# lukeshope/hipims-ocl

Hardware: AMD Instinct MI355X
Metric: Mcell-steps/sec fp64 Godunov+HLLC, 4096^2 grid, 1/2/4/8 MI355X; % HBM roofline (higher is better)
Workload: dtype f64

## Files before the change

### hipims-ocl_amd/csrc/hp_domain.hpp

```cpp
#pragma once
#include "../../include/hipims_mi.h"
#include "hp_facts.hpp"
#include "hp_plan.hpp"
#include "hp_kernels.hpp"
#include "hp_peaks.hpp"
#include "hp_probes.hpp"
#include "hp_zones.hpp"
#include "hp_overview.hpp"
#include "hp_sparse.hpp"
#include "hp_bed.hpp"
#include "hp_links.hpp"
#include "hp_soil.hpp"
#include <rccl/rccl.h>

#include <algorithm>
#include <atomic>
#include <string>
#include <vector>

using namespace hp;

namespace {

thread_local std::string g_last_error;
// ... 190 lines not shown
	uint64_t         peer_rounds = 0;
	void*            peer_state[2][2] = {{nullptr, nullptr}, {nullptr, nullptr}};
	long             peer_rows[2] = {0, 0};
	unsigned*        push_arrived = nullptr;
	bool             peer_direct = false;
	bool             push_now = false;
	unsigned long long* tail_words = nullptr;
	bool             fill_now = false;
	void*            z_state = nullptr;
	unsigned long long* haz_words = nullptr;
	unsigned         pair_gen = 0;
	void*            still_rec = nullptr;
	size_t           still_rec_slots = 0;
	int              still_rec_half = 0;
	bool             still_rec_last = false;
	uint64_t         pair_cold_starts = 0;
	hipEvent_t       tune_ev[4] = {nullptr, nullptr, nullptr, nullptr};
	int              tune_phase = 0;
	bool             tune_prefer_pairs = true;
	uint64_t         tune_next = 0;
	uint64_t         tune_samples = 0, tune_switches = 0;
	float            tune_pair_ms = 0.f, tune_single_ms = 0.f;
	uint64_t         pairs = 0;
	unsigned         single_streak = 0;
	uint64_t         flux_launches = 0, flux_launches_tailed = 0;
	bool             tail_failed = false;
	bool             strip_first = false;
	bool             tail_allowed = false;
	bool             tail_want = false;
	int              tail_fresh = 0;
	bool             tail_done = false;
	bool             spec_now = false;
	uint32_t         spec_pending = 0;
	void*            spec_state = nullptr;
	void*            spec_scalars = nullptr;
	struct { int adv_fresh; uint64_t cells_calculated, iterations; } spec_host;
	uint64_t         spec_batches = 0, spec_replays = 0;
	OutputStage      out;
	PeakTracker      peaks;
	ProbeRecorder    probes;
	ZoneRecorder     zones;
	BedShapes        beds;
	LinkStore        links;
	SoilStore        soil;
};

// ... 41 lines not shown
```

### hipims-ocl_amd/csrc/hp_engine.hip

```cpp
#include "hp_domain.hpp"
#include "hp_observers.hpp"
#include "hp_actors.hpp"
#include <hip/hip_ext.h>
#include <dlfcn.h>

#include <algorithm>
#include <cmath>
#include <cstdio>
#include <cstdlib>
#include <cstring>
#include <random>
#include <string>
#include <vector>
#include <unistd.h>

namespace {

constexpr size_t CFL_SLOT_BYTES = 1024;

struct Rccl {
	void* handle = nullptr;
	decltype(&ncclGetUniqueId)   GetUniqueId = nullptr;
	decltype(&ncclCommInitRank)  CommInitRank = nullptr;
	decltype(&ncclCommDestroy)   CommDestroy = nullptr;
// ... 7 lines not shown
	std::string path;
} g_rccl;

void peer_release(hp_domain* d);
PeerBox peer_box(hp_domain* d, bool use, long timeout_ms = 0);
PeerPush make_push(const hp_domain* d);

const PlanKnobs& plan_knobs()
{
	static const PlanKnobs knobs = [] {
		auto num = [](const char* name, int unset) { const char* e = std::getenv(name); return e ? std::atoi(e) : unset; };
		auto off = [&](const char* name) { return num(name, 1) == 0; };
		auto on = [&](const char* name) { return num(name, 0) != 0; };
		auto force = [&](const char* name) { return std::getenv(name) ? (num(name, 0) != 0 ? 1 : 0) : -1; };
		PlanKnobs k;
		k.two_step = num("HP_TWO_STEP", -1);
		k.launch_tail = !off("HP_LAUNCH_TAIL"); k.strip_reduce_always = on("HP_STRIP_REDUCE_ALWAYS");
		k.pair_bdy = !off("HP_PAIR_BDY"); k.pair_strict = !off("HP_PAIR_STRICT"); k.pair_exact = force("HP_PAIR_EXACT");
		k.pair_skip = !off("HP_PAIR_SKIP"); k.fill_after_pairs = !off("HP_FILL_AFTER_PAIRS");
		k.strict_speculate = on("HP_STRICT_SPECULATE"); k.pair_tune = !off("HP_PAIR_TUNE"); k.sweep_alternate = force("HP_SWEEP_ALTERNATE");
		k.tail_max_blocks = (unsigned)num("HP_TAIL_MAX_BLOCKS", (int)TAIL_MAX_BLOCKS);
		k.tail_max_blocks_k2k6 = (unsigned)num("HP_TAIL_MAX_BLOCKS_K2K6", (int)TAIL_MAX_BLOCKS);
		k.march2_rseg_forced = std::getenv("HP_MARCH2_RSEG") != nullptr;
		k.fuse_bdy = !off("HP_FUSE_BDY");
		return k;
	}();
	return knobs;
}
PlanDomain plan_domain(const hp_domain* d)
{
	PlanDomain p;
	p.scheme = d->desc.scheme; p.kernel = d->desc.kernel; p.math_mode = d->desc.math_mode; p.precision = d->desc.precision; p.dynamic_dt = d->desc.dynamic_dt;
	p.quirks = d->desc.quirks; p.rows = d->desc.rows; p.cols = d->desc.cols; p.cells = d->cells;
	p.row_offset = d->desc.row_offset; p.global_rows = d->desc.global_rows; p.ghost_rows = d->ghost_rows;
	p.has_bdy = !d->bdy.empty(); p.fusable = d->fusable; p.bdy_on_ring = d->bdy_on_ring;
	for (const Boundary& b : d->bdy)
		if ((b.kind == BDY_UNIFORM && b.definition == HP_UNIFORM_LOSS_RATE) || (b.kind == BDY_GRIDDED && b.definition == HP_GRIDDED_MASS_FLUX)) p.bdy_removes_water = true;
	p.has_comm = d->comm != nullptr; p.comm_world = d->comm_world; p.peer_direct = d->peer_direct; p.peer_mine = d->peer_mine != nullptr;
	p.has_tail_words = d->tail_words != nullptr; p.tail_allowed = d->tail_allowed; p.halo_overlap = d->halo_overlap; p.split_now = d->split_now;
	p.strip_any_bdy = d->strip_any_bdy; p.strip_first = d->strip_first; p.strip_any_full = d->strip_any_full;
	p.spec_now = d->spec_now; p.has_stamps = d->z_state != nullptr; p.march2_pays = d->tiling.march2_pays;
	p.has_links = d->links.groups != 0; p.soil_on = d->soil.on;
#ifdef HP_KEEP_SPEC_FUSED
	p.spec_fused_kept = true;
#endif
	return p;
}

template <typename T> Params<T> make_params(const hp_domain* d)
{
	Params<T> p;
	p.cols = d->desc.cols; p.rows = d->desc.rows;
	p.row_offset = d->desc.row_offset; p.global_rows = d->desc.global_rows;
	p.dx = (T)d->desc.dx;
	p.inv_dx = T(1) / p.dx;
	p.vs = (T)d->desc.dry_threshold;
	p.qs = (T)d->desc.dry_threshold * T(10);
	p.courant = (T)d->desc.courant;
	p.t_end = (T)d->desc.t_end;
	p.dt_fixed = (T)d->desc.dt_fixed;
	p.friction = d->desc.friction;
	p.dynamic_dt = d->desc.dynamic_dt;
	p.manning_uniform = d->manning_uniform ? 1 : 0;
	p.manning_value = (T)d->manning_value;
// ... 434 lines not shown
	const size_t slots = (size_t)windows * (size_t)d->desc.rows;
	if (d->still_rec && d->still_rec_slots == slots) return HP_OK;
	hipFree(d->still_rec);
	d->still_rec = nullptr;
	d->facts.buffers_written_outside();
	const size_t bytes = (2 * slots + 1) * sizeof(StillRec);
	HIP_TRY(hipMalloc(&d->still_rec, bytes));
	HIP_TRY(hipMemsetAsync(d->still_rec, 0xff, bytes, d->stream));
	d->still_rec_slots = slots;
	return HP_OK;
}
template <typename T> int pair_cold_start(hp_domain* d)
{
	int rc;
	d->facts.buffers_written_outside();
	if ((rc = apply_boundaries<T>(d, d->state[0])) != HP_OK) return rc;
	if ((rc = launch_reduce<T>(d, d->state[0], d->own_lo, d->own_hi)) != HP_OK) return rc;
	hipLaunchKernelGGL((pair_cold_start_words<T>), dim3(1), dim3(1), 0, d->stream, (T*)d->cfl_slot);
	HIP_TRY(hipGetLastError());
	d->facts.cold_started();
	d->pair_cold_starts++;
	return HP_OK;
}
template <typename T> int run_pair_t(hp_domain* d, const bool strip, const bool followed)
{
	const Params<T> p = make_params<T>(d);
	TileMap tm;
	unsigned blocks;
	long lo, hi;
	if (strip) {
		const bool south = d->desc.row_offset > 0, north = d->desc.row_offset + d->desc.rows < d->desc.global_rows;
		lo = south ? d->ghost_rows : 1;
		hi = d->desc.rows - (north ? d->ghost_rows : 1);
	} else launch_rows(d, 1, lo, hi);
	const PlanDomain pd = plan_domain(d);
	const PlanKnobs& knobs = plan_knobs();
	const int rseg2 = pair_tile_rows(pd, knobs, d->tiling.march2_rseg);
	if (!make_tile_map(launch_knobs(), lo, hi, 1, PART_ALL, (int)((p.cols - 2 + MARCH2_COLS - 1) / MARCH2_COLS), rseg2, rseg2, 0, tm, blocks, rseg2,
	                   0, d->own_lo, d->own_hi, d->tiling.march2_nbands))
		return HP_ERR_STATE;
	if (blocks > tail_limit(knobs)) return HP_ERR_STATE;
	d->tail_want = true; d->tail_allowed = true; d->push_now = strip;
	d->tail_fresh = strip ? (d->desc.dynamic_dt ? 7 : 4) : (d->desc.dynamic_dt ? 1 : 0);
	d->tail_done = false;
	LaunchTail<T> tail;
	const int kind = make_tail<T>(d, blocks, PART_ALL, d->stream, tail_limit(knobs), tail);
	d->tail_want = false; d->tail_allowed = false; d->push_now = false;
	if (kind != (strip ? 2 : 1)) return HP_ERR_STATE;
	const bool bdy = pd.has_bdy;
	int rc;
	if ((rc = pair_stamps_alloc(d)) != HP_OK) return rc;
	bool in_place = false;
	if (bdy && !d->facts->m1_valid) {
		if ((rc = pair_cold_start<T>(d)) != HP_OK) return rc;
		in_place = true;
	} else if (bdy) in_place = d->facts->pair_fused_next;
	tail.pair = bdy ? 2 : 1;
	tail.bdy_flag = bdy && followed ? 1 : 0;
	PairAux<T> aux{};
	const bool exact = pair_exact(pd, knobs) && d->z_state != nullptr;
	if (exact) aux.stamps = StampBufs<T>{(char*)d->z_state, d->haz_words};
	aux.prev_gen = d->facts->other_stale ? d->pair_gen : 0u;
	aux.gen = ++d->pair_gen;
	if (aux.gen == 0) aux.gen = ++d->pair_gen;
	aux.list = (const AreaBdyList<T>*)d->fused_list; aux.fuse_next = bdy && followed ? 1 : 0; aux.in_place = in_place ? 1 : 0;
	aux.truncated = (d->desc.quirks & HP_QUIRK_BDY_TRUNCATED) != 0 ? 1 : 0;
	const bool recs = pair_records(pd, knobs, strip, exact, rseg2);
	if (recs) {
		if ((rc = still_rec_alloc(d, tm.nstrips)) != HP_OK) return rc;
		StillRec* const base = (StillRec*)d->still_rec;
		aux.still_out = base + (size_t)(d->still_rec_half ^ 1) * d->still_rec_slots;
		aux.still_in = d->facts->still_rec_valid ? base + (size_t)d->still_rec_half * d->still_rec_slots : nullptr;
		aux.still_rows = d->desc.rows;
	}
	const void* src = d->state[0];
	void* dst = d->state[1];
	const bool sample = d->timing_stride > 0 && d->timing_used < d->timing_events.size() &&
	                    (d->timing_counter++ % (uint64_t)d->timing_stride) == 0;
	if (sample) HIP_TRY(hipEventRecord(d->timing_events[d->timing_used].first, d->stream));
#define HP_LAUNCH_K1B2(CFL_, BDY_, HZ_, TAIL_)                                                                                            \
	hipLaunchKernelGGL((godunov_march2<false, CFL_, BDY_, HZ_, TAIL_, T>), dim3(blocks), dim3(256), 0, d->stream, p, (const Scalars<T>*)d->scalars, \
	                   (const T*)d->bed, (const State4<T>*)src, (State4<T>*)dst, (const T*)d->manning, (T*)d->cfl_slot,                    \
	                   (const T*)d->cfl_slot + SLOT_EDGE, tm, tail, aux)
#define HP_LAUNCH_K1B(CFL_, BDY_, TAIL_) do { if (exact) HP_LAUNCH_K1B2(CFL_, BDY_, true, TAIL_); else HP_LAUNCH_K1B2(CFL_, BDY_, false, TAIL_); } while (0)
	if (d->desc.math_mode == HP_MATH_STRICT)
		hipLaunchKernelGGL((godunov_march2<true, 1, false, true, 1, T>), dim3(blocks), dim3(256), 0, d->stream, p, (const Scalars<T>*)d->scalars,
		                   (const T*)d->bed, (const State4<T>*)src, (State4<T>*)dst, (const T*)d->manning, (T*)d->cfl_slot,
		                   (const T*)d->cfl_slot + SLOT_EDGE, tm, tail, aux);
	else
	if (strip)    { if (d->desc.dynamic_dt) HP_LAUNCH_K1B2(1, false, false, 2); else HP_LAUNCH_K1B2(0, false, false, 2); }
	else if (bdy) HP_LAUNCH_K1B(1, true, 1);
	else          { if (d->desc.dynamic_dt) HP_LAUNCH_K1B(1, false, 1); else HP_LAUNCH_K1B(0, false, 1); }
#undef HP_LAUNCH_K1B
#undef HP_LAUNCH_K1B2
	d->facts.pair_queued(bdy, followed);
	HIP_TRY(hipGetLastError());
	if (recs) d->still_rec_half ^= 1;
	d->facts.pair_launched(recs); d->still_rec_last = recs;
	if (sample) { HIP_TRY(hipEventRecord(d->timing_events[d->timing_used].second, d->stream)); d->timing_used++; }
	std::swap(d->state[0], d->state[1]);
	if (strip) {
		std::swap(d->peer_state[0][0], d->peer_state[0][1]);
		std::swap(d->peer_state[1][0], d->peer_state[1][1]);
	}
	d->facts.pair_ran(strip, d->ghost_rows);
	d->single_streak = 0;
	d->tail_done = false; d->fork_is_advance = false;
	d->adv_fresh = d->desc.dynamic_dt ? 1 : 0;
	d->cells_calculated += 2 * (uint64_t)d->desc.cols * (uint64_t)d->desc.rows;
	d->iterations += 2;
	d->pairs += 1;
	return HP_OK;
}
static int run_pair(hp_domain* d, const bool strip = false, const bool followed = false)
{
	return d->desc.precision == 8 ? run_pair_t<double>(d, strip, followed) : run_pair_t<float>(d, strip, followed);
}
static int repair_other_buffer(hp_domain* d)
{
	if (!d->facts->other_stale) return HP_OK;
	d->facts.buffers_written_outside();
	HIP_TRY(hipMemcpyAsync(d->state[d->facts->use_alt ^ 1], d->state[d->facts->use_alt], d->cells * 4 * d->esize, hipMemcpyDeviceToDevice, d->stream));
	if (d->z_state) {
		if (d->desc.precision == 8)
			hipLaunchKernelGGL((stamps_to_buffer<double>), dim3(1024), dim3(256), 0, d->stream, (State4<double>*)d->state[d->facts->use_alt ^ 1],
			                   StampBufs<double>{(char*)d->z_state, d->haz_words}, d->pair_gen, d->cells);
		else
			hipLaunchKernelGGL((stamps_to_buffer<float>), dim3(1024), dim3(256), 0, d->stream, (State4<float>*)d->state[d->facts->use_alt ^ 1],
			                   StampBufs<float>{(char*)d->z_state, d->haz_words}, d->pair_gen, d->cells);
		HIP_TRY(hipGetLastError());
	}
	d->facts.other_made_current();
	return HP_OK;
}
static int snapshot_take(hp_domain* d, void* state, void* scalars, const int first)
{
	const size_t bytes = d->cells * 4 * d->esize;
	const size_t sc_bytes = d->desc.precision == 8 ? sizeof(Scalars<double>) : sizeof(Scalars<float>);
	HIP_TRY(hipMemcpyAsync(state, d->state[first], bytes, hipMemcpyDeviceToDevice, d->stream));
// ... 522 lines not shown
			if ((rc = pair_stamps_alloc(d)) != HP_OK) return rc;
			rc = run_pair(d, false, true);
			if (rc == HP_OK) {
				HIP_TRY(hipEventRecord(d->tune_ev[0], d->stream));
				if ((rc = run_pair(d, false, true)) != HP_OK || (rc = run_pair(d, false, true)) != HP_OK) return rc;
				HIP_TRY(hipEventRecord(d->tune_ev[1], d->stream));
				if ((rc = repair_other_buffer(d)) != HP_OK) return rc;
				if ((rc = run_single(d, true)) != HP_OK || (rc = run_single(d, true)) != HP_OK) return rc;
				HIP_TRY(hipEventRecord(d->tune_ev[2], d->stream));
				for (int k = 0; k < 4; ++k)
					if ((rc = run_single(d, k < 3 || i + 12 < n_iterations)) != HP_OK) return rc;
				HIP_TRY(hipEventRecord(d->tune_ev[3], d->stream));
				d->tune_phase = 1;
				i += 11;
				continue;
			}
			if (rc != HP_ERR_STATE) return rc;
		}
		if (i + 2 <= n_iterations && (!tune || d->tune_prefer_pairs) && pair_eligible(plan_domain(d), d->facts, plan_knobs())) {
			rc = run_pair(d, false, i + 2 < n_iterations);
			if (rc == HP_OK) { ++i; continue; }
			if (rc != HP_ERR_STATE) return rc;
		}
		if ((rc = run_single(d, i + 1 < n_iterations)) != HP_OK) return rc;
	}
	d->fuse_next = 0;
	return HP_OK;
}
int spec_resolve(hp_domain* d)
{
	const uint32_t n = d->spec_pending;
	d->spec_pending = 0;
	HIP_TRY(hipStreamSynchronize(d->stream));
	static const long force = std::getenv("HP_STRICT_SPEC_FORCE") ? std::atol(std::getenv("HP_STRICT_SPEC_FORCE")) : 0;
	const double flag = *(volatile double*)((char*)d->host_scalars + HOST_SPEC_FLAG);
	const bool raised = flag != 0.0 || (force > 0 && d->spec_batches % (uint64_t)force == 0);
	if (!raised) return HP_OK;
	d->spec_replays++;
	log_line(HP_LOG_INFORMATION, "a speculative STRICT batch of " + std::to_string(n) + " iterations is re-run with the plain divisions");
	const size_t bytes = d->cells * 4 * d->esize, sc_bytes = sizeof(Scalars<double>);
	d->facts.buffers_written_outside();
	HIP_TRY(hipMemcpyAsync(d->state[0], d->spec_state, bytes, hipMemcpyDeviceToDevice, d->stream));
	HIP_TRY(hipMemcpyAsync(d->state[1], (char*)d->spec_state + bytes, bytes, hipMemcpyDeviceToDevice, d->stream));
	HIP_TRY(hipMemcpyAsync(d->scalars, d->spec_scalars, sc_bytes, hipMemcpyDeviceToDevice, d->stream));
	HIP_TRY(hipMemcpyAsync(d->cfl_slot, (char*)d->spec_scalars + sc_bytes, CFL_SLOT_BYTES, hipMemcpyDeviceToDevice, d->stream));
	d->facts.spec_replayed();
// ... 722 lines not shown
	double total = 0.0;
	uint32_t n = 0;
	for (size_t i = 0; i < d->timing_used; ++i) {
		float ms = 0.f;
		HIP_TRY(hipEventElapsedTime(&ms, d->timing_events[i].first, d->timing_events[i].second));
		total += std::max(0.0, (double)ms - d->timing_overhead_ms);
		++n;
	}
	*avg_ms = n ? total / n : 0.0;
	*samples = n;
	return HP_OK;
}

int hp_pair_stats(hp_domain_t* d, uint64_t out[12])
{
	int rc = check_domain(d);
	if (rc != HP_OK) return rc;
	if (!out) return fail(HP_ERR_INVALID, "out == NULL");
	out[0] = d->pairs; out[1] = d->pair_cold_starts; out[2] = out[3] = 0;
	HIP_TRY(hipStreamSynchronize(d->stream));
	if (tuner_on(plan_domain(d), plan_knobs()) && (rc = tuner_poll(d)) != HP_OK) return rc;
	out[4] = d->tune_samples; out[5] = d->tune_switches; out[6] = d->tune_prefer_pairs ? 1 : 0;
	out[7] = d->tune_single_ms > 0.f ? (uint64_t)(1000.0 * d->tune_pair_ms / d->tune_single_ms) : 0;
	out[8] = out[9] = out[10] = out[11] = 0;
	if (d->still_rec && d->still_rec_last) {
		const StillRec* half = (const StillRec*)d->still_rec + (size_t)d->still_rec_half * d->still_rec_slots;
		unsigned long long* counts = (unsigned long long*)((StillRec*)d->still_rec + 2 * d->still_rec_slots);
		HIP_TRY(hipMemsetAsync(counts, 0, 16, d->stream));
		hipLaunchKernelGGL(still_rec_count, dim3(256), dim3(256), 0, d->stream, half, d->still_rec_slots, counts);
		HIP_TRY(hipGetLastError());
		unsigned long long host_counts[2] = {0, 0};
		HIP_TRY(hipMemcpyAsync(host_counts, counts, sizeof host_counts, hipMemcpyDeviceToHost, d->stream));
		HIP_TRY(hipStreamSynchronize(d->stream));
		out[9] = host_counts[0]; out[10] = host_counts[1];
	}
	if (d->haz_words) {
		unsigned long long used = 0;
		HIP_TRY(hipMemcpy(&used, d->haz_words + 2, sizeof used, hipMemcpyDeviceToHost));
		out[8] = used;
	}
	if (!d->z_state) return HP_OK;
	unsigned long long* counts = d->haz_words + 4;
	HIP_TRY(hipMemsetAsync(counts, 0, 16, d->stream));
	if (d->desc.precision == 8)
		hipLaunchKernelGGL((stamps_count<double>), dim3(1024), dim3(256), 0, d->stream, StampBufs<double>{(char*)d->z_state, d->haz_words}, d->pair_gen, d->cells, counts);
	else
		hipLaunchKernelGGL((stamps_count<float>), dim3(1024), dim3(256), 0, d->stream, StampBufs<float>{(char*)d->z_state, d->haz_words}, d->pair_gen, d->cells, counts);
// ... 29 lines not shown
```

### hipims-ocl_amd/csrc/hp_kernels.hpp

```cpp
#pragma once

#include "hp_math.hpp"
#include "hp_tiling.hpp"

namespace hp {

template <bool STRICT, typename T>
__global__ __launch_bounds__(256) void godunov_basic(const Params<T> p, const Scalars<T>* __restrict__ sc,
                                                     const T* __restrict__ bed, const State4<T>* __restrict__ src,
                                                     State4<T>* __restrict__ dst, const T* __restrict__ manning,
                                                     const long y_lo, const long y_hi)
{
	const long x = (long)blockIdx.x * blockDim.x + threadIdx.x;
	const long y = (long)blockIdx.y * blockDim.y + threadIdx.y + y_lo;
	if (x >= p.cols - 1 || y >= y_hi || x <= 0) return;
	const size_t id = (size_t)y * p.cols + x;
	const T dt = sc->dt;

	if (dt <= T(0)) { dst[id] = src[id]; return; }

	const State4<T> c = src[id];
	const T zb = bed[id], n = manning[id];
	if (c.zmax <= T(-9999.0) || c.z == T(-9999.0)) { dst[id] = c; return; }

// ... 836 lines not shown
				}
				if (FUSED && fuse) {
					const State4<T> rained = apply_fused(c, zb, y);
					dst[id] = rained;
					if (TAIL == 2) store_peer(rained, y, true);
				}
			}
		}
	}

	if (CFL_MODE != 0) {
		if (blockIdx.x == 0 && wave == 0) { const T e = *edge_max; if (e > vmax) vmax = e; }
		vmax = wave_max(vmax);
		if (TAIL != 0) wave_vmax = vmax;
		else if (lane == 0 && vmax > T(0)) atomic_max_nonneg(cfl_slot, vmax);
	}
	if (FUSED && blockIdx.x == 0 && wave == 0 && lane == 0) cfl_slot[SLOT_BDY] = fuse_flag ? T(1) : T(0);
	}
	if (TAIL != 0) tail_block_done(tail, wave_vmax, wave, lane, y0, y1);
}

template <typename T> struct RowU1 { State4<T> c; T zb; bool plain; };

template <bool STRICT, int CFL_MODE, bool BDY, bool HZ, int TAIL, typename T>
#ifndef HP_K1B_WAVES_MIN
#define HP_K1B_WAVES_MIN 3
#endif
#ifndef HP_K1B_F32_WAVES_MIN
#define HP_K1B_F32_WAVES_MIN 5
#endif
#ifndef HP_K1B_F32_WAVES_MAX
#define HP_K1B_F32_WAVES_MAX 5
#endif
__global__ __launch_bounds__(256) __attribute__((amdgpu_waves_per_eu(sizeof(T) == 4 ? (STRICT ? 3 : (HZ ? 4 : HP_K1B_F32_WAVES_MIN)) : (STRICT ? HP_K1B_STRICT_WAVES : HP_K1B_WAVES_MIN), sizeof(T) == 4 ? (STRICT ? 3 : HP_K1B_F32_WAVES_MAX) : (STRICT ? HP_K1B_STRICT_WAVES : 3)))) void godunov_march2(
	const Params<T> p, const Scalars<T>* sc, const T* __restrict__ bed, const State4<T>* __restrict__ src,
	State4<T>* __restrict__ dst, const T* __restrict__ manning, T* cfl_slot, const T* __restrict__ edge_max,
	const TileMap tm, const LaunchTail<T> tail, const PairAux<T> aux)
{
	if (TAIL != 0 && blockIdx.x >= tail.flux_blocks) {
		launch_tail(p, tail);
		return;
	}
	__shared__ T inc_tab[BDY ? 4 * 3 * FUSED_BDY_MAX * 2 * 64 : 1];
	const int lane = threadIdx.x & 63, wave = __builtin_amdgcn_readfirstlane((int)(threadIdx.x >> 6));
	long strip, y0, y1;
	T wave_vmax = T(0), wave_vmax1 = T(0);
	if (tile_rows(tm, wave, strip, y0, y1)) {

	const long x = strip * MARCH2_COLS - 1 + lane;
	const long xc = x < 0 ? 0 : (x < p.cols ? x : (p.cols - 1));
	const bool out_x = lane >= 2 && lane <= MARCH2_COLS + 1 && x <= p.cols - 2;
	const bool ring_x = x <= 0 || x >= p.cols - 1;
	const T vs = p.vs;
	const bool with_friction = p.friction != 0;
	const T inv_dx = STRICT ? p.inv_dx_pow2 : p.inv_dx;

	Scalars<T> s1 = *sc;
	const Scalars<T> s0 = s1;
	const T dt_a = s1.dt;
	advance_scalars(p, s1, p.dynamic_dt ? cfl_slot[BDY ? SLOT_M1 : SLOT_SAVED] : T(0));
	const T dt_b = s1.dt;
	const bool skip_a = dt_a <= T(0), skip_b = dt_b <= T(0);
	constexpr bool SCALAR_CONSTS = !STRICT && sizeof(T) == 8;
	constexpr bool HIDE = BDY || HZ;
	const StepConsts<T> ka{uniform_value<HIDE>(-(dt_a * p.inv_dx)), uniform_value<HIDE>(dt_a * gravity<T>()), SCALAR_CONSTS};
	const StepConsts<T> kb{uniform_value<HIDE>(-(dt_b * p.inv_dx)), uniform_value<HIDE>(dt_b * gravity<T>()), SCALAR_CONSTS};

	const long row_base = y0 - 2 < 0 ? 0 : y0 - 2, col_base = strip * MARCH2_COLS - 1 < 0 ? 0 : strip * MARCH2_COLS - 1;
	const size_t cell0 = (size_t)row_base * p.cols + (size_t)col_base;
	const size_t cells_left = (size_t)p.cols * p.rows - cell0;
	const __amdgpu_buffer_rsrc_t srd_src = make_srd(src + cell0, cells_left * sizeof(State4<T>));
	const __amdgpu_buffer_rsrc_t srd_dst = make_srd(dst + cell0, cells_left * sizeof(State4<T>));
	const __amdgpu_buffer_rsrc_t srd_bed = make_srd(bed + cell0, cells_left * sizeof(T));
	const __amdgpu_buffer_rsrc_t srd_man = make_srd(manning + cell0, cells_left * sizeof(T));
	const unsigned lane_col = (unsigned)(xc - col_base);
	const unsigned voff_state = lane_col * (unsigned)sizeof(State4<T>), voff_scalar = lane_col * (unsigned)sizeof(T);
	const unsigned row_state = (unsigned)p.cols * (unsigned)sizeof(State4<T>), row_scalar = (unsigned)p.cols * (unsigned)sizeof(T);
	const long last_row = p.rows - 1;
	const __amdgpu_buffer_rsrc_t srd_peer0 = make_srd((TAIL == 2 && tail.peer_rows[0] ? tail.peer_rows[0] : dst) + cell0, cells_left * sizeof(State4<T>));
	const __amdgpu_buffer_rsrc_t srd_peer1 = make_srd((TAIL == 2 && tail.peer_rows[1] ? tail.peer_rows[1] : dst) + cell0, cells_left * sizeof(State4<T>));
	auto store_peer = [&](const State4<T>& v, const long y, const bool write_lane) {
		const bool e0 = (int)y >= tail.edge_rows[0] && (int)y < tail.edge_rows[1];
		const bool e1 = (int)y >= tail.edge_rows[2] && (int)y < tail.edge_rows[3];
		buf_store_state<HP_AUX_THROUGH>(v, e1 ? srd_peer1 : srd_peer0, (write_lane && (e0 || e1)) ? voff_state : HP_OOB, (unsigned)(y - row_base) * row_state);
	};
// ... 417 lines not shown
			const unsigned row_k = (unsigned)__builtin_amdgcn_readfirstlane((int)(yy - row_base));
			buf_store_state(c, srd_dst, out_x ? voff_state : HP_OOB, row_k * row_state);
			if (TAIL == 2) store_peer(c, yy, out_x);
			if (CFL_MODE == 1 && out_x && (int)yy >= tm.price_lo && (int)yy < tm.price_hi && spd > vmax) vmax = spd;
		};
		State4<T> a = q[2].c, b = q[3].c;
		for (;;) {
			if (y >= y1) return y;
			#pragma unroll
			for (int j = 0; j < 4; ++j) q[j] = load_rz(y + 2 + j);
			if (!in_run(q[0])) return y;
			put(a, y);
			if (y + 1 >= y1 || !in_run(q[1])) return y + 1;
			put(b, y + 1);
			if (y + 2 >= y1 || !in_run(q[2])) return y + 2;
			put(q[0].c, y + 2);
			if (y + 3 >= y1 || !in_run(q[3])) return y + 3;
			put(q[1].c, y + 3);
			a = q[2].c; b = q[3].c;
			y += 4;
		}
	};

	const long yb = (RUNS && !skip_a && !skip_b) ? still_run() : y0;
	write_recs(STILL_TAG_RUN);
	if (!RUNS || yb < y1) {
		prime(yb);
		long r = yb + 1;
		for (; r + 1 <= y1; r += 2) {
			{ const T nn = rc.n; const RowU1<T> u = stage_a(r, rP, rQ); stage_b(r - 1, u, nn, true); }
			{ const T nn = rc.n; const RowU1<T> u = stage_a(r + 1, rQ, rP); stage_b(r, u, nn, true); }
		}
		if (r <= y1) { const T nn = rc.n; const RowU1<T> u = stage_a(r, rP, rQ); stage_b(r - 1, u, nn, true); }
	}

	if (wave_any(stale_rows != 0)) {
		for (long y = y0; y < y1; ++y) {
			if ((stale_rows >> (unsigned)(y - y0)) & 1u) {
				const size_t id = (size_t)y * p.cols + xc;
				const T zb = bed[id];
				State4<T> c = src[id];
				if (live0) c = apply(J0(), c, zb, y);
				State4<T> next = c;
				if (live2) next = apply(J2(), c, zb, y);
				dst[id] = fuse ? next : c;
				if (TAIL == 2) store_peer(fuse ? next : c, y, true);
				if (CFL_MODE == 1 && (int)y >= tm.price_lo && (int)y < tm.price_hi) {
					const T s = cfl_speed<STRICT>(c.z, c.zmax, c.qx, c.qy, zb, p.qs);
					if (s > vmax) vmax = s;
					if (live2) {
						const T s2 = cfl_speed<STRICT>(next.z, next.zmax, next.qx, next.qy, zb, p.qs);
						if (s2 > vmax1) vmax1 = s2;
					}
				}
			}
		}
	}
	if (!live2) vmax1 = vmax;
	};

	auto raise_word = [&]() { if (hz_on && wave_any(stamped) && lane == 0) aux.stamps.haz[aux.gen & 1u] = (unsigned long long)aux.gen; };
	if (RECS && aux.still_in != nullptr && !skip_a && !skip_b && tile_known()) {
		still_marks = ~0u;
		write_recs(STILL_TAG_SKIP);
		if (CFL_MODE == 1 && out_x && (int)y1 > tm.price_lo && (int)y0 < tm.price_hi)
			vmax = cfl_speed<STRICT>(T(__longlong_as_double((long long)still_kz)), T(0), T(0), T(0), T(__longlong_as_double((long long)still_kb)), p.qs);
		vmax1 = vmax;
	} else {
	if (BDY && act != 0) { if (hz_any) march(std::true_type(), std::true_type()); else march(std::true_type(), std::false_type()); }
	else                 { if (hz_any) march(std::false_type(), std::true_type()); else march(std::false_type(), std::false_type()); }
	raise_word();
	}

	if (CFL_MODE != 0) {
		if (blockIdx.x == 0 && wave == 0) { const T e = *edge_max; if (e > vmax) vmax = e; if (e > vmax1) vmax1 = e; }
		vmax = wave_max(vmax);
		if (BDY) vmax1 = wave_max(vmax1);
		if (TAIL != 0) { wave_vmax = vmax; wave_vmax1 = vmax1; }
		else if (lane == 0 && vmax > T(0)) atomic_max_nonneg(cfl_slot, vmax);
	}
	}
	if (TAIL != 0) tail_block_done<BDY>(tail, wave_vmax, wave, lane, y0, y1, wave_vmax1);
}

template <typename T>
__global__ __launch_bounds__(256) void stamps_to_buffer(State4<T>* __restrict__ other, const StampBufs<T> b, const unsigned gen, const size_t cells)
{
	if (b.haz[gen & 1u] != (unsigned long long)gen) return;
	for (size_t id = (size_t)blockIdx.x * blockDim.x + threadIdx.x; id < cells; id += (size_t)gridDim.x * blockDim.x)
		if (stamp_gen(b, id) == gen) other[id] = stamp_state(b, id);
}

template <typename T>
__global__ __launch_bounds__(256) void stamps_count(const StampBufs<T> b, const unsigned gen, const size_t cells, unsigned long long* counts)
{
	unsigned long long last = 0, any = 0;
	for (size_t id = (size_t)blockIdx.x * blockDim.x + threadIdx.x; id < cells; id += (size_t)gridDim.x * blockDim.x) {
		const unsigned g = stamp_gen(b, id);
		last += (g != 0 && g == gen); any += (g != 0);
	}
	for (int off = 32; off > 0; off >>= 1) { last += __shfl_down(last, off); any += __shfl_down(any, off); }
	if ((threadIdx.x & 63) == 0 && (last | any)) { atomicAdd(counts, last); atomicAdd(counts + 1, any); }
}
__global__ __launch_bounds__(256) void still_rec_count(const StillRec* __restrict__ rec, const size_t n, unsigned long long* counts)
{
// ... 636 lines not shown
```

### hipims-ocl_amd/csrc/hp_plan.hpp

```cpp
#pragma once
#include "../../include/hipims_mi.h"
#include "hp_facts.hpp"

#include <algorithm>
#include <cstddef>
#include <cstdint>

namespace hp {
namespace {

constexpr unsigned TAIL_MAX_BLOCKS = 65536;
constexpr uint32_t SPEC_MIN = 8;

struct PlanKnobs {
	int      two_step = -1;
	bool     launch_tail = true;
	bool     strip_reduce_always = false;
	bool     pair_bdy = true;
	bool     pair_strict = true;
	int      pair_exact = -1;
	bool     pair_skip = true;
	bool     fill_after_pairs = true;
	bool     strict_speculate = false;
	bool     pair_tune = true;
	int      sweep_alternate = -1;
	unsigned tail_max_blocks = TAIL_MAX_BLOCKS;
	unsigned tail_max_blocks_k2k6 = TAIL_MAX_BLOCKS;
	bool     march2_rseg_forced = false;
	bool     fuse_bdy = true;
};

struct PlanDomain {
	int      scheme = HP_SCHEME_GODUNOV, kernel = HP_KERNEL_AUTO, math_mode = HP_MATH_FAST, precision = 8, dynamic_dt = 1;
	unsigned quirks = HP_QUIRKS_REFERENCE;
	long     rows = 0, cols = 0;
	size_t   cells = 0;
	long     row_offset = 0, global_rows = 0, ghost_rows = 1;
	bool     has_bdy = false;
	bool     fusable = false, bdy_on_ring = false;
	bool     bdy_removes_water = false;
	bool     has_comm = false;
	int      comm_world = 1;
	bool     peer_direct = false, peer_mine = false;
	bool     has_tail_words = true, tail_allowed = false, halo_overlap = false, split_now = true;
	bool     strip_any_bdy = false, strip_first = false, strip_any_full = false;
	bool     spec_now = false;
	bool     has_stamps = false;
	bool     march2_pays = false;
	bool     has_links = false, soil_on = false;
	bool     spec_fused_kept = false;
};

inline bool reads_primary(const PlanDomain& d) { return (d.quirks & HP_QUIRK_CFL_READS_PRIMARY) != 0; }
inline bool basic_godunov(const PlanDomain& d) { return d.kernel == HP_KERNEL_BASIC && d.scheme == HP_SCHEME_GODUNOV; }
inline bool boundaries_applied(const PlanDomain& d) { return d.has_bdy && d.scheme != HP_SCHEME_MUSCL_HANCOCK; }

inline unsigned tail_limit(const PlanKnobs& k) { return k.tail_max_blocks < TAIL_MAX_BLOCKS ? k.tail_max_blocks : TAIL_MAX_BLOCKS; }
inline unsigned tail_limit_k2k6(const PlanKnobs& k) { return std::min(tail_limit(k), k.tail_max_blocks_k2k6); }
inline int tail_kind_for(const bool tail_want, const bool part_all, const bool own_stream, const unsigned blocks, const unsigned limit, const bool push_now)
{
	if (!(tail_want && part_all && own_stream && blocks <= limit)) return 0;
	return push_now ? 2 : 1;
}

inline bool sweep_alternates(const PlanDomain& d, const PlanKnobs& k)
{
	if (k.sweep_alternate >= 0) return k.sweep_alternate != 0;
	return d.precision == 4 || d.scheme == HP_SCHEME_MUSCL_HANCOCK;
}

inline bool pairs_possible_common(const PlanDomain& d, const PlanKnobs& k)
// ... 14 lines not shown
	       d.global_rows == d.rows;
}
inline bool pair_eligible(const PlanDomain& d, const BufferFacts& facts, const PlanKnobs& k)
{
	return pairs_possible(d, k) && facts.pair_ready(d.dynamic_dt != 0);
}
inline bool strip_pairs_possible_here(const PlanDomain& d, const BufferFacts& facts, const PlanKnobs& k)
{
	return pairs_possible_common(d, k) && d.has_comm && d.comm_world > 1 && d.peer_direct && d.ghost_rows == 2 && !facts->rings_differ;
}
inline bool pair_exact(const PlanDomain& d, const PlanKnobs& k)
{
	if (d.math_mode == HP_MATH_STRICT) return true;
	if (k.pair_exact >= 0) return k.pair_exact != 0;
	return d.bdy_removes_water;
}
inline int pair_tile_rows(const PlanDomain& d, const PlanKnobs& k, const int march2_rseg)
{
	return (d.math_mode == HP_MATH_STRICT && !k.march2_rseg_forced) ? std::min(march2_rseg, 12) : march2_rseg;
}
inline bool pair_records(const PlanDomain& d, const PlanKnobs& k, const bool strip, const bool exact, const int tile_rows)
{
	return d.precision == 8 && k.pair_skip && !strip && !d.has_bdy && !exact && d.math_mode != HP_MATH_STRICT && tile_rows <= 32;
}

inline bool fill_wanted(const PlanDomain& d, const BufferFacts& facts, const PlanKnobs& k)
{
	return k.fill_after_pairs && facts->other_stale && d.scheme == HP_SCHEME_GODUNOV && d.kernel != HP_KERNEL_BASIC && !(pair_exact(d, k) && d.has_stamps);
}

inline bool spec_wanted(const PlanDomain& d, const PlanKnobs& k, const uint32_t n)
{
	const bool fusable_ok = d.spec_fused_kept || !d.fusable;
	return k.strict_speculate && n >= SPEC_MIN && d.math_mode == HP_MATH_STRICT && d.precision == 8 && !d.has_comm && fusable_ok && !d.has_links && !d.soil_on &&
	       d.kernel != HP_KERNEL_BASIC && (d.scheme == HP_SCHEME_GODUNOV || d.scheme == HP_SCHEME_MUSCL_HANCOCK);
}
inline bool tuner_on(const PlanDomain& d, const PlanKnobs& k)
{
	return k.pair_tune && d.math_mode == HP_MATH_STRICT && k.two_step != 1;
}

inline bool strips_reduce_everyone(const PlanDomain& d, const BufferFacts& facts, const bool first_of_batch)
{
	const bool dst_is_primary = facts->use_alt == 1;
	return d.dynamic_dt && (d.scheme == HP_SCHEME_MUSCL_HANCOCK || !reads_primary(d) || dst_is_primary || basic_godunov(d) || d.strip_any_bdy ||
	                        (first_of_batch && d.strip_any_full));
// ... 45 lines not shown
```

### hipims-ocl_amd/hipims_mi/__init__.py

```python
from __future__ import annotations

import ctypes as C
import os
import weakref

import numpy as np

HERE = os.path.dirname(os.path.abspath(__file__))
PKG_ROOT = os.path.dirname(HERE)
LIB_PATH = os.path.join(PKG_ROOT, "lib", "libhipims_mi.so")

SCHEME_GODUNOV, SCHEME_MUSCL_HANCOCK, SCHEME_INERTIAL = 0, 1, 2
ARRAY_STATE, ARRAY_BED, ARRAY_MANNING = 0, 1, 2
QUIRK_CFL_READS_PRIMARY, QUIRK_BDY_TRUNCATED, QUIRK_MUSCL_NEIGHBOUR_Y_IS_BED, QUIRKS_REFERENCE = 1, 2, 4, 7
MATH_FAST, MATH_STRICT = 0, 1
KERNEL_AUTO, KERNEL_BASIC = 0, 1
UNIFORM_RAIN_INTENSITY, UNIFORM_LOSS_RATE = 0, 1
GRIDDED_RAIN_INTENSITY, GRIDDED_RAIN_ACCUMUL, GRIDDED_MASS_FLUX = 0, 1, 2
DEPTH_IGNORE, DEPTH_IS_FSL, DEPTH_IS_DEPTH, DEPTH_IS_CRITICAL = 0, 1, 2, 3
DISCHARGE_IGNORE, DISCHARGE_IS_DISCHARGE, DISCHARGE_IS_VELOCITY, DISCHARGE_IS_VOLUME = 0, 1, 2, 3
PTR_STATE_NEXT_SRC, PTR_STATE_OTHER, PTR_BED, PTR_MANNING, PTR_CFL_MAX, PTR_SCALARS = range(6)
(OUT_DEPTH, OUT_MAXDEPTH, OUT_FSL, OUT_MAXFSL, OUT_DISCHARGE_X, OUT_DISCHARGE_Y, OUT_VELOCITY_X, OUT_VELOCITY_Y, OUT_FROUDE,
 OUT_COUNT) = range(10)
OUT_CODES = {"depth": OUT_DEPTH, "maxdepth": OUT_MAXDEPTH, "fsl": OUT_FSL, "maxfsl": OUT_MAXFSL, "dischargex": OUT_DISCHARGE_X,
# ... 1012 lines not shown
    def kernel_timing(self, stride):
        _check(self.lib, self.lib.hp_kernel_timing(self.h, stride), "hp_kernel_timing")

    def kernel_timing_read(self):
        avg, n = C.c_double(0), C.c_uint32(0)
        _check(self.lib, self.lib.hp_kernel_timing_read(self.h, C.byref(avg), C.byref(n)), "hp_kernel_timing_read")
        return avg.value, n.value

    def launch_counts(self):
        if not hasattr(self.lib, "hp_launch_counts"):
            return None
        a, b = C.c_uint64(0), C.c_uint64(0)
        _check(self.lib, self.lib.hp_launch_counts(self.h, C.byref(a), C.byref(b)), "hp_launch_counts")
        return a.value, b.value

    def pair_stats(self):
        if not hasattr(self.lib, "hp_pair_stats"):
            return None
        out = (C.c_uint64 * 12)()
        self.lib.hp_pair_stats.argtypes = [C.c_void_p, C.POINTER(C.c_uint64)]
        _check(self.lib, self.lib.hp_pair_stats(self.h, out), "hp_pair_stats")
        return dict(pairs=out[0], cold_starts=out[1], stamped_last=out[2], stamped_ever=out[3], tune_samples=out[4],
                    tune_switches=out[5], prefers_pairs=bool(out[6]), pair_over_single=out[7] / 1000.0, stale_used=out[8],
                    skipped_rows=out[9], still_rows=out[10])

    def kernel_timing_overhead(self):
        if not hasattr(self.lib, "hp_kernel_timing_overhead"):
            return 0.0
        ms = C.c_double(0)
        _check(self.lib, self.lib.hp_kernel_timing_overhead(self.h, C.byref(ms)), "hp_kernel_timing_overhead")
        return ms.value

    def depth_velocity(self, state=None, bed=None):
        state = self.download() if state is None else state
        bed = self._bed_host if bed is None else bed
        depth = np.maximum(0.0, state[..., 0].astype(np.float64) - bed.astype(np.float64))
        with np.errstate(divide="ignore", invalid="ignore"):
            u = np.where(depth > 1e-8, state[..., 2] / depth, 0.0)
            v = np.where(depth > 1e-8, state[..., 3] / depth, 0.0)
        return depth, u, v
```

Measured before the change: 121,900.

## Run trailing odd single step through the pair kernel with still-region skipping

When a batch ends on an odd iteration, the final single step now runs through a one-step variant of the fused two-step march kernel instead of the generic single-step path. The point is to let that step use the still-record skipping and tail reduction machinery that paired steps already have, so quiescent rows are skipped. This adds a new kernel instantiation and a separate bookkeeping path for buffer facts and CFL state, which could diverge from what the single-step path maintains. It only applies when there are no boundaries and no strips, the fp64 non-strict mode is in use, and the other buffer is stale.

```diff
diff --git a/hipims-ocl_amd/csrc/hp_domain.hpp b/hipims-ocl_amd/csrc/hp_domain.hpp
--- a/hipims-ocl_amd/csrc/hp_domain.hpp
+++ b/hipims-ocl_amd/csrc/hp_domain.hpp
@@ -236,6 +236,7 @@
 	uint64_t         tune_samples = 0, tune_switches = 0;
 	float            tune_pair_ms = 0.f, tune_single_ms = 0.f;
 	uint64_t         pairs = 0;
+	uint64_t         one_steps = 0;
 	unsigned         single_streak = 0;
 	uint64_t         flux_launches = 0, flux_launches_tailed = 0;
 	bool             tail_failed = false;
diff --git a/hipims-ocl_amd/csrc/hp_engine.hip b/hipims-ocl_amd/csrc/hp_engine.hip
--- a/hipims-ocl_amd/csrc/hp_engine.hip
+++ b/hipims-ocl_amd/csrc/hp_engine.hip
@@ -53,7 +53,7 @@
 		k.tail_max_blocks = (unsigned)num("HP_TAIL_MAX_BLOCKS", (int)TAIL_MAX_BLOCKS);
 		k.tail_max_blocks_k2k6 = (unsigned)num("HP_TAIL_MAX_BLOCKS_K2K6", (int)TAIL_MAX_BLOCKS);
 		k.march2_rseg_forced = std::getenv("HP_MARCH2_RSEG") != nullptr;
-		k.fuse_bdy = !off("HP_FUSE_BDY");
+		k.fuse_bdy = !off("HP_FUSE_BDY"); k.one_step = !off("HP_ONE_STEP");
 		return k;
 	}();
 	return knobs;
@@ -70,7 +70,7 @@
 	p.has_comm = d->comm != nullptr; p.comm_world = d->comm_world; p.peer_direct = d->peer_direct; p.peer_mine = d->peer_mine != nullptr;
 	p.has_tail_words = d->tail_words != nullptr; p.tail_allowed = d->tail_allowed; p.halo_overlap = d->halo_overlap; p.split_now = d->split_now;
 	p.strip_any_bdy = d->strip_any_bdy; p.strip_first = d->strip_first; p.strip_any_full = d->strip_any_full;
-	p.spec_now = d->spec_now; p.has_stamps = d->z_state != nullptr; p.march2_pays = d->tiling.march2_pays;
+	p.spec_now = d->spec_now; p.has_stamps = d->z_state != nullptr; p.march2_pays = d->tiling.march2_pays; p.march2_rseg = d->tiling.march2_rseg;
 	p.has_links = d->links.groups != 0; p.soil_on = d->soil.on;
 #ifdef HP_KEEP_SPEC_FUSED
 	p.spec_fused_kept = true;
@@ -551,7 +551,7 @@
 	d->pair_cold_starts++;
 	return HP_OK;
 }
-template <typename T> int run_pair_t(hp_domain* d, const bool strip, const bool followed)
+template <typename T> int run_pair_t(hp_domain* d, const bool strip, const bool followed, const bool one_step)
 {
 	const Params<T> p = make_params<T>(d);
 	TileMap tm;
@@ -569,8 +569,12 @@
 	                   0, d->own_lo, d->own_hi, d->tiling.march2_nbands))
 		return HP_ERR_STATE;
 	if (blocks > tail_limit(knobs)) return HP_ERR_STATE;
+	const SinglePlan lone = plan_single(pd, d->facts, knobs);
+	if (one_step && (strip || pd.has_bdy || lone.reprice_ring || lone.reduce_after || lone.cfl_mode == 2 ||
+	                 !pair_records(pd, knobs, strip, pair_exact(pd, knobs), rseg2)))
+		return HP_ERR_STATE;
 	d->tail_want = true; d->tail_allowed = true; d->push_now = strip;
-	d->tail_fresh = strip ? (d->desc.dynamic_dt ? 7 : 4) : (d->desc.dynamic_dt ? 1 : 0);
+	d->tail_fresh = one_step ? lone.tail_fresh : strip ? (d->desc.dynamic_dt ? 7 : 4) : (d->desc.dynamic_dt ? 1 : 0);
 	d->tail_done = false;
 	LaunchTail<T> tail;
 	const int kind = make_tail<T>(d, blocks, PART_ALL, d->stream, tail_limit(knobs), tail);
@@ -584,7 +588,7 @@
 		if ((rc = pair_cold_start<T>(d)) != HP_OK) return rc;
 		in_place = true;
 	} else if (bdy) in_place = d->facts->pair_fused_next;
-	tail.pair = bdy ? 2 : 1;
+	tail.pair = one_step ? 0 : (bdy ? 2 : 1);
 	tail.bdy_flag = bdy && followed ? 1 : 0;
 	PairAux<T> aux{};
 	const bool exact = pair_exact(pd, knobs) && d->z_state != nullptr;
@@ -602,9 +606,9 @@
 		aux.still_in = d->facts->still_rec_valid ? base + (size_t)d->still_rec_half * d->still_rec_slots : nullptr;
 		aux.still_rows = d->desc.rows;
 	}
-	const void* src = d->state[0];
-	void* dst = d->state[1];
-	const bool sample = d->timing_stride > 0 && d->timing_used < d->timing_events.size() &&
+	const void* src = d->state[one_step ? d->facts->use_alt : 0];
+	void* dst = d->state[one_step ? d->facts->use_alt ^ 1 : 1];
+	const bool sample = !one_step && d->timing_stride > 0 && d->timing_used < d->timing_events.size() &&
 	                    (d->timing_counter++ % (uint64_t)d->timing_stride) == 0;
 	if (sample) HIP_TRY(hipEventRecord(d->timing_events[d->timing_used].first, d->stream));
 #define HP_LAUNCH_K1B2(CFL_, BDY_, HZ_, TAIL_)                                                                                            \
@@ -612,6 +616,16 @@
 	                   (const T*)d->bed, (const State4<T>*)src, (State4<T>*)dst, (const T*)d->manning, (T*)d->cfl_slot,                    \
 	                   (const T*)d->cfl_slot + SLOT_EDGE, tm, tail, aux)
 #define HP_LAUNCH_K1B(CFL_, BDY_, TAIL_) do { if (exact) HP_LAUNCH_K1B2(CFL_, BDY_, true, TAIL_); else HP_LAUNCH_K1B2(CFL_, BDY_, false, TAIL_); } while (0)
+	if (one_step) {
+		if constexpr (sizeof(T) == 8) {
+			if (d->desc.dynamic_dt)
+				hipLaunchKernelGGL((godunov_march2_one<1, T>), dim3(blocks), dim3(256), 0, d->stream, p, (const Scalars<T>*)d->scalars, (const T*)d->bed, (const State4<T>*)src,
+				                   (State4<T>*)dst, (const T*)d->manning, (T*)d->cfl_slot, (const T*)d->cfl_slot + SLOT_EDGE + lone.edge_buffer, tm, tail, aux);
+			else
+				hipLaunchKernelGGL((godunov_march2_one<0, T>), dim3(blocks), dim3(256), 0, d->stream, p, (const Scalars<T>*)d->scalars, (const T*)d->bed, (const State4<T>*)src,
+				                   (State4<T>*)dst, (const T*)d->manning, (T*)d->cfl_slot, (const T*)d->cfl_slot + SLOT_EDGE + lone.edge_buffer, tm, tail, aux);
+		}
+	} else
 	if (d->desc.math_mode == HP_MATH_STRICT)
 		hipLaunchKernelGGL((godunov_march2<true, 1, false, true, 1, T>), dim3(blocks), dim3(256), 0, d->stream, p, (const Scalars<T>*)d->scalars,
 		                   (const T*)d->bed, (const State4<T>*)src, (State4<T>*)dst, (const T*)d->manning, (T*)d->cfl_slot,
@@ -622,10 +636,21 @@
 	else          { if (d->desc.dynamic_dt) HP_LAUNCH_K1B(1, false, 1); else HP_LAUNCH_K1B(0, false, 1); }
 #undef HP_LAUNCH_K1B
 #undef HP_LAUNCH_K1B2
-	d->facts.pair_queued(bdy, followed);
+	if (one_step) d->facts.single_begins(); else d->facts.pair_queued(bdy, followed);
 	HIP_TRY(hipGetLastError());
 	if (recs) d->still_rec_half ^= 1;
 	d->facts.pair_launched(recs); d->still_rec_last = recs;
+	if (one_step) {
+		d->facts.other_made_current();
+		if (d->desc.dynamic_dt && lone.cfl_mode != 0) d->facts.maximum_priced();
+		d->facts.single_ended();
+		d->tail_done = false; d->fork_is_advance = false;
+		d->adv_fresh = (d->desc.dynamic_dt && lone.cfl_mode != 0) ? 1 : 0;
+		d->cells_calculated += (uint64_t)d->desc.cols * (uint64_t)d->desc.rows;
+		d->iterations += 1;
+		d->one_steps += 1;
+		return HP_OK;
+	}
 	if (sample) { HIP_TRY(hipEventRecord(d->timing_events[d->timing_used].second, d->stream)); d->timing_used++; }
 	std::swap(d->state[0], d->state[1]);
 	if (strip) {
@@ -641,9 +666,9 @@
 	d->pairs += 1;
 	return HP_OK;
 }
-static int run_pair(hp_domain* d, const bool strip = false, const bool followed = false)
-{
-	return d->desc.precision == 8 ? run_pair_t<double>(d, strip, followed) : run_pair_t<float>(d, strip, followed);
+static int run_pair(hp_domain* d, const bool strip = false, const bool followed = false, const bool one_step = false)
+{
+	return d->desc.precision == 8 ? run_pair_t<double>(d, strip, followed, one_step) : run_pair_t<float>(d, strip, followed, one_step);
 }
 static int repair_other_buffer(hp_domain* d)
 {
@@ -1212,6 +1237,11 @@
 			if (rc == HP_OK) { ++i; continue; }
 			if (rc != HP_ERR_STATE) return rc;
 		}
+		if (i + 1 == n_iterations && single_as_one_step(plan_domain(d), d->facts, plan_knobs())) {
+			rc = run_pair(d, false, false, true);
+			if (rc == HP_OK) continue;
+			if (rc != HP_ERR_STATE) return rc;
+		}
 		if ((rc = run_single(d, i + 1 < n_iterations)) != HP_OK) return rc;
 	}
 	d->fuse_next = 0;
@@ -1980,7 +2010,7 @@
 	if (tuner_on(plan_domain(d), plan_knobs()) && (rc = tuner_poll(d)) != HP_OK) return rc;
 	out[4] = d->tune_samples; out[5] = d->tune_switches; out[6] = d->tune_prefer_pairs ? 1 : 0;
 	out[7] = d->tune_single_ms > 0.f ? (uint64_t)(1000.0 * d->tune_pair_ms / d->tune_single_ms) : 0;
-	out[8] = out[9] = out[10] = out[11] = 0;
+	out[8] = out[9] = out[10] = 0; out[11] = d->one_steps;
 	if (d->still_rec && d->still_rec_last) {
 		const StillRec* half = (const StillRec*)d->still_rec + (size_t)d->still_rec_half * d->still_rec_slots;
 		unsigned long long* counts = (unsigned long long*)((StillRec*)d->still_rec + 2 * d->still_rec_slots);
diff --git a/hipims-ocl_amd/csrc/hp_kernels.hpp b/hipims-ocl_amd/csrc/hp_kernels.hpp
--- a/hipims-ocl_amd/csrc/hp_kernels.hpp
+++ b/hipims-ocl_amd/csrc/hp_kernels.hpp
@@ -882,7 +882,6 @@
 
 template <typename T> struct RowU1 { State4<T> c; T zb; bool plain; };
 
-template <bool STRICT, int CFL_MODE, bool BDY, bool HZ, int TAIL, typename T>
 #ifndef HP_K1B_WAVES_MIN
 #define HP_K1B_WAVES_MIN 3
 #endif
@@ -892,7 +891,8 @@
 #ifndef HP_K1B_F32_WAVES_MAX
 #define HP_K1B_F32_WAVES_MAX 5
 #endif
-__global__ __launch_bounds__(256) __attribute__((amdgpu_waves_per_eu(sizeof(T) == 4 ? (STRICT ? 3 : (HZ ? 4 : HP_K1B_F32_WAVES_MIN)) : (STRICT ? HP_K1B_STRICT_WAVES : HP_K1B_WAVES_MIN), sizeof(T) == 4 ? (STRICT ? 3 : HP_K1B_F32_WAVES_MAX) : (STRICT ? HP_K1B_STRICT_WAVES : 3)))) void godunov_march2(
+template <bool STRICT, int CFL_MODE, bool BDY, bool HZ, int TAIL, typename T, bool ONE_STEP>
+__device__ __forceinline__ void godunov_march2_body(
 	const Params<T> p, const Scalars<T>* sc, const T* __restrict__ bed, const State4<T>* __restrict__ src,
 	State4<T>* __restrict__ dst, const T* __restrict__ manning, T* cfl_slot, const T* __restrict__ edge_max,
 	const TileMap tm, const LaunchTail<T> tail, const PairAux<T> aux)
@@ -920,7 +920,8 @@
 	const T dt_a = s1.dt;
 	advance_scalars(p, s1, p.dynamic_dt ? cfl_slot[BDY ? SLOT_M1 : SLOT_SAVED] : T(0));
 	const T dt_b = s1.dt;
-	const bool skip_a = dt_a <= T(0), skip_b = dt_b <= T(0);
+	static_assert(!ONE_STEP || (!STRICT && !BDY && !HZ && TAIL == 1 && sizeof(T) == 8), "one-step launches: the instantiations with still records");
+	const bool skip_a = dt_a <= T(0), skip_b = ONE_STEP || dt_b <= T(0);
 	constexpr bool SCALAR_CONSTS = !STRICT && sizeof(T) == 8;
 	constexpr bool HIDE = BDY || HZ;
 	const StepConsts<T> ka{uniform_value<HIDE>(-(dt_a * p.inv_dx)), uniform_value<HIDE>(dt_a * gravity<T>()), SCALAR_CONSTS};
@@ -1384,7 +1385,7 @@
 		}
 	};
 
-	const long yb = (RUNS && !skip_a && !skip_b) ? still_run() : y0;
+	const long yb = (RUNS && !skip_a && (ONE_STEP || !skip_b)) ? still_run() : y0;
 	write_recs(STILL_TAG_RUN);
 	if (!RUNS || yb < y1) {
 		prime(yb);
@@ -1422,7 +1423,7 @@
 	};
 
 	auto raise_word = [&]() { if (hz_on && wave_any(stamped) && lane == 0) aux.stamps.haz[aux.gen & 1u] = (unsigned long long)aux.gen; };
-	if (RECS && aux.still_in != nullptr && !skip_a && !skip_b && tile_known()) {
+	if (RECS && aux.still_in != nullptr && !skip_a && (ONE_STEP || !skip_b) && tile_known()) {
 		still_marks = ~0u;
 		write_recs(STILL_TAG_SKIP);
 		if (CFL_MODE == 1 && out_x && (int)y1 > tm.price_lo && (int)y0 < tm.price_hi)
@@ -1443,6 +1444,22 @@
 	}
 	}
 	if (TAIL != 0) tail_block_done<BDY>(tail, wave_vmax, wave, lane, y0, y1, wave_vmax1);
+}
+template <bool STRICT, int CFL_MODE, bool BDY, bool HZ, int TAIL, typename T>
+__global__ __launch_bounds__(256) __attribute__((amdgpu_waves_per_eu(sizeof(T) == 4 ? (STRICT ? 3 : (HZ ? 4 : HP_K1B_F32_WAVES_MIN)) : (STRICT ? HP_K1B_STRICT_WAVES : HP_K1B_WAVES_MIN), sizeof(T) == 4 ? (STRICT ? 3 : HP_K1B_F32_WAVES_MAX) : (STRICT ? HP_K1B_STRICT_WAVES : 3)))) void godunov_march2(
+	const Params<T> p, const Scalars<T>* sc, const T* __restrict__ bed, const State4<T>* __restrict__ src,
+	State4<T>* __restrict__ dst, const T* __restrict__ manning, T* cfl_slot, const T* __restrict__ edge_max,
+	const TileMap tm, const LaunchTail<T> tail, const PairAux<T> aux)
+{
+	godunov_march2_body<STRICT, CFL_MODE, BDY, HZ, TAIL, T, false>(p, sc, bed, src, dst, manning, cfl_slot, edge_max, tm, tail, aux);
+}
+template <int CFL_MODE, typename T>
+__global__ __launch_bounds__(256) __attribute__((amdgpu_waves_per_eu(HP_K1B_WAVES_MIN, 3))) void godunov_march2_one(
+	const Params<T> p, const Scalars<T>* sc, const T* __restrict__ bed, const State4<T>* __restrict__ src,
+	State4<T>* __restrict__ dst, const T* __restrict__ manning, T* cfl_slot, const T* __restrict__ edge_max,
+	const TileMap tm, const LaunchTail<T> tail, const PairAux<T> aux)
+{
+	godunov_march2_body<false, CFL_MODE, false, false, 1, T, true>(p, sc, bed, src, dst, manning, cfl_slot, edge_max, tm, tail, aux);
 }
 
 template <typename T>
diff --git a/hipims-ocl_amd/csrc/hp_plan.hpp b/hipims-ocl_amd/csrc/hp_plan.hpp
--- a/hipims-ocl_amd/csrc/hp_plan.hpp
+++ b/hipims-ocl_amd/csrc/hp_plan.hpp
@@ -28,6 +28,7 @@
 	unsigned tail_max_blocks_k2k6 = TAIL_MAX_BLOCKS;
 	bool     march2_rseg_forced = false;
 	bool     fuse_bdy = true;
+	bool     one_step = true;
 };
 
 struct PlanDomain {
@@ -47,6 +48,7 @@
 	bool     spec_now = false;
 	bool     has_stamps = false;
 	bool     march2_pays = false;
+	int      march2_rseg = 24;
 	bool     has_links = false, soil_on = false;
 	bool     spec_fused_kept = false;
 };
@@ -107,6 +109,12 @@
 inline bool pair_records(const PlanDomain& d, const PlanKnobs& k, const bool strip, const bool exact, const int tile_rows)
 {
 	return d.precision == 8 && k.pair_skip && !strip && !d.has_bdy && !exact && d.math_mode != HP_MATH_STRICT && tile_rows <= 32;
+}
+
+inline bool single_as_one_step(const PlanDomain& d, const BufferFacts& facts, const PlanKnobs& k)
+{
+	return k.one_step && pairs_possible(d, k) && pair_records(d, k, false, pair_exact(d, k), pair_tile_rows(d, k, d.march2_rseg)) &&
+	       facts.pair_ready(d.dynamic_dt != 0) && facts->other_stale;
 }
 
 inline bool fill_wanted(const PlanDomain& d, const BufferFacts& facts, const PlanKnobs& k)
diff --git a/hipims-ocl_amd/hipims_mi/__init__.py b/hipims-ocl_amd/hipims_mi/__init__.py
--- a/hipims-ocl_amd/hipims_mi/__init__.py
+++ b/hipims-ocl_amd/hipims_mi/__init__.py
@@ -1058,7 +1058,7 @@
         _check(self.lib, self.lib.hp_pair_stats(self.h, out), "hp_pair_stats")
         return dict(pairs=out[0], cold_starts=out[1], stamped_last=out[2], stamped_ever=out[3], tune_samples=out[4],
                     tune_switches=out[5], prefers_pairs=bool(out[6]), pair_over_single=out[7] / 1000.0, stale_used=out[8],
-                    skipped_rows=out[9], still_rows=out[10])
+                    skipped_rows=out[9], still_rows=out[10], one_steps=out[11])
 
     def kernel_timing_overhead(self):
         if not hasattr(self.lib, "hp_kernel_timing_overhead"):
```

Result: no change. 122,400 (median of 6 runs) (+0.4%).
